# lilinitsy/skele-raytracer

Hardware: AMD Instinct MI355X
Metric: Mrays/sec + frame ms, 1920x1080 gillum=16 spheres2.scn (higher is better)
Workload: dtype f32

## Files before the change

skele_raytracer_amd/csrc/launch.h:

```cpp
#pragma once

#include <hip/hip_runtime.h>
#include <stddef.h>
#include <stdint.h>

#include "render_params.h"

enum { SKR_LEVEL0_RUN = 0, SKR_LEVEL0_BUILD, SKR_LEVEL0_REPLAY };
enum { SKR_PIX_NONE = 0, SKR_PIX_NODE, SKR_PIX_BACKGROUND, SKR_PIX_TRIANGLE };

constexpr int SKR_NODE_LEVELS_MAX = 33;
struct NodePlan {
	bool flat = false;
	int levels = 0;
	uint32_t band_nblk = 0;
	uint64_t nodes_max[SKR_NODE_LEVELS_MAX] = {};
	uint32_t cap[SKR_NODE_LEVELS_MAX] = {};
	size_t off_nodes[SKR_NODE_LEVELS_MAX] = {}, off_shade[SKR_NODE_LEVELS_MAX] = {}, off_recs[SKR_NODE_LEVELS_MAX] = {}, off_res[SKR_NODE_LEVELS_MAX] = {}, off_ixh[SKR_NODE_LEVELS_MAX] = {};
	size_t off_ctr = 0, ctr_bytes = 0, total = 0, banded = 0;
	size_t off_cls = 0, off_sums = 0;
	size_t off_girow = 0;
	int level0 = SKR_LEVEL0_RUN;
	size_t lds_leaf = 0;
	size_t lds = 0;
};

constexpr int SKR_GLEVELS_MAX = 64;
struct GPlan {
	int levels = 0;
	uint32_t band_rows = 0;
	uint64_t nodes_max[SKR_GLEVELS_MAX + 1] = {};
	uint32_t cap[SKR_GLEVELS_MAX + 1] = {};
	size_t off_nodes[SKR_GLEVELS_MAX + 1] = {}, off_recs[SKR_GLEVELS_MAX + 1] = {}, off_res[SKR_GLEVELS_MAX + 1] = {}, off_hdr[SKR_GLEVELS_MAX + 1] = {};
	size_t off_ctr = 0, ctr_bytes = 0, total = 0;
};

struct QueryTrees {
	const float4 *tree;
	const float4 *trace;
	uint32_t stride;
	int32_t nchunks;
	int32_t cones, trace_cones;
	float4 ball;
};

// ... 48 lines not shown
constexpr size_t SKR_PREFIX_LDS = ((size_t) SKR_PREFIX_WORDS * sizeof(uint32_t) + 15) & ~(size_t) 15;
static inline size_t skr_scene_kernels_lds(const RenderParams &p) { return skr_scene_lds_bytes(p) + 32 + SKR_PREFIX_LDS; }
static inline size_t skr_lights_lds_bytes(const RenderParams &p) { return ((size_t) 1 + 2 * p.n_lights) * 16; }
static inline size_t skr_lights_kernels_lds(const RenderParams &p) { return skr_lights_lds_bytes(p) + 32 + SKR_PREFIX_LDS; }

static inline uint32_t skr_tree_arity(const RenderParams &p) { return (uint32_t) (p.monte_carlo ? p.num_path_traces : 0) + (p.legacy_reflect ? 2u * (uint32_t) p.n_lights : 0u); }

struct ScratchLayout {
	size_t off = 0;
	size_t take(size_t bytes) { const size_t o = off; off += (bytes + 255) & ~(size_t) 255; return o; }
};

template <class Fits>
static uint32_t skr_largest_band(uint32_t all, Fits fits)
{
	if(fits(all)) return all;
	uint32_t lo = 1, hi = all;
	if(!fits(lo)) return 0;
	while(hi - lo > 1)
	{
		const uint32_t mid = lo + (hi - lo) / 2;
		if(fits(mid)) lo = mid;
		else hi = mid;
	}
	return lo;
}

#ifndef SKR_TRACE_BY_NODE
#define SKR_TRACE_BY_NODE 1
#endif
#ifndef SKR_TRACE_RUN
#define SKR_TRACE_RUN 2
#endif
__host__ __device__ static inline uint64_t skr_trace_header_row(uint64_t node, uint32_t j, uint32_t PP)
{
	return SKR_TRACE_BY_NODE ? (node >> 6) * PP + j : (node * PP + j) >> 6;
}
__host__ __device__ static inline uint32_t skr_trace_header_bit(uint64_t node, uint32_t j, uint32_t PP)
{
	return (uint32_t) (SKR_TRACE_BY_NODE ? node : node * PP + j) & 63u;
}
static inline uint64_t skr_trace_rows_used(uint64_t nodes, uint64_t PP) { return SKR_TRACE_BY_NODE ? (nodes + 63) / 64 * PP : (nodes * PP + 63) / 64; }
static inline uint64_t skr_trace_rows_alloc(uint64_t nodes, uint64_t PP) { return skr_trace_rows_used(nodes, PP) + 4; }
static inline uint64_t skr_trace_region_cap(uint64_t nodes, uint64_t PP) { return (skr_trace_rows_used(nodes, PP) + SKR_P1_REGIONS - 1) / SKR_P1_REGIONS * 128; }

enum SkrLeafShape { SKR_LEAF_RUNTIME = 0, SKR_LEAF_POINT1 = 1, SKR_LEAF_POINT2 = 2 };
static inline SkrLeafShape skr_leaf_shape(const RenderParams &p)
{
	if(!(p.sw.shadow_mask & SKR_SW_LEAF_SHAPE)) return SKR_LEAF_RUNTIME;
	if(p.n_tris != 0 || p.gi_index == nullptr || p.gi_wide != 0) return SKR_LEAF_RUNTIME;
	if(!p.use_shadows || p.shadow_masks == nullptr) return SKR_LEAF_RUNTIME;
	if(p.pow_steps > 7) return SKR_LEAF_RUNTIME;
	return p.n_lights == 2 ? SKR_LEAF_POINT2 : p.n_lights == 1 ? SKR_LEAF_POINT1 : SKR_LEAF_RUNTIME;
}

bool skr_plan_launch(const RenderParams &p, size_t lds_limit, LaunchPlan &lp, const GenericFeatures &f);
const char *skr_features_conflict(const GenericFeatures &f, bool legacy_reflect, bool shade_triangles, bool fog);
const char *skr_generic_variant(bool query, const GenericFeatures &f);
hipError_t skr_launch_render(const RenderParams &p, const LaunchPlan &lp, hipStream_t stream, const SkrTimingHook *hook);
hipError_t skr_launch_debug(int op, const void *d_in, void *d_out, uint32_t n, hipStream_t stream);
bool skr_nodes_plan(const RenderParams &p, size_t lds_limit, NodePlan &pl);
hipError_t skr_launch_nodes(const RenderParams &p, const NodePlan &pl, hipStream_t stream, const SkrTimingHook *hook);
hipError_t skr_nodes_level_count(const void *scratch, size_t off_ctr, int level, uint32_t *n);
bool skr_generic_plan(const RenderParams &p, GPlan &pl, bool sphere_tree = false);
hipError_t skr_launch_generic(const RenderParams &p, const GPlan &pl, hipStream_t stream, const SkrTimingHook *hook, const GenericFeatures &f, const ShadeRays *q = nullptr);
struct PrimaryKey {
// ... 65 lines not shown
```

skele_raytracer_amd/csrc/render_nodes.hip:

```cpp
#include <hip/hip_runtime.h>
#include <stdint.h>
#include <stdlib.h>
#include <string.h>

#include <vector>

#include "launch.h"
#include "wave_common.h"

namespace {

constexpr uint32_t PC_HIT0 = 1u, PC_HIT1 = 2u, PC_BLACK0 = 4u, PC_BLACK1 = 8u;
constexpr int IXH_ROWS = 3;
constexpr int NQ_CAP = 176;
constexpr int NQ_PRE = NQ_CAP - 128;
constexpr int NQ_F = 5;
constexpr int NWIN = 4;
constexpr int WIN_FLOATS = 2 * 3 * 64;
constexpr int LEAF2_WAVE_FLOATS = NQ_CAP * NQ_F + NWIN * WIN_FLOATS;

typedef const RenderParams __attribute__((address_space(4))) *LaunchArgs;
SKR_DEV const RenderParams &launch_args()
{
	LaunchArgs k = (LaunchArgs) __builtin_amdgcn_kernarg_segment_ptr();
// ... 2 lines not shown
}

SKR_DEV bool classify_child(const SceneView &sv, f3 co, f3 d, float two_a, float four_a, const BestState &s, bool &black)
{
	black = false;
	if(sv.nt > 0)
	{
		const float tmin = (s.best >= 0) ? near_root(two_a, s.b, s.D) : __builtin_inff();
		black = any_triangle_closer(sv, RayConst{co, d, two_a, four_a}, tmin);
	}
	return !black && s.best >= 0;
}

}

#ifndef SKR_TRACE_LOOP
#define SKR_TRACE_LOOP 1
#endif
#if SKR_TRACE_LOOP
#define SKR_TRACE_STRIDE gridDim.x
#else
#define SKR_TRACE_STRIDE 0x40000000u
#undef SKR_TRACE_GRID_MAX
#define SKR_TRACE_GRID_MAX 0x7fffffffu
#endif
#ifndef SKR_TRACE_WAVES
#define SKR_TRACE_WAVES 0
#endif
#if SKR_TRACE_WAVES
#define SKR_TRACE_ATTR __attribute__((amdgpu_waves_per_eu(SKR_TRACE_WAVES, SKR_TRACE_WAVES)))
#else
#define SKR_TRACE_ATTR
#endif
template <bool TRIS, bool GIM>
SKR_DEV void trace_round(const SceneView &sv, const RenderParams &p, bool valid, uint32_t node, uint32_t j, f3 co, f3 Nn, f3 nt, f3 nb, uint32_t pixel,
						 uint32_t node_id, int gi_row, uint32_t chunk, int lane, Counters &cn)
{
	const uint32_t N = (uint32_t) p.num_path_traces;
	const bool second = valid && 2u * j + 1u < N;
	bool hit0 = false, hit1 = false;
	float4 rec0 = make_float4(0, 0, 0, 0), rec1 = rec0;
	bool black0 = false, black1 = false;
	if(valid)
	{
		uint32_t rnd[4];
		philox4x32(pixel, p.aa_index, node_id, j, p.seed_lo, p.seed_hi, rnd);
		const float q1a = u31_to_unit(rnd[0]), q2a = u31_to_unit(rnd[1]), q1b = u31_to_unit(rnd[2]), q2b = u31_to_unit(rnd[3]);
		const DirPair dp = gi_direction_pair(q1a, q2a, q1b, q2b, Nn, nt, nb);
		const f3 d0 = dp.d0, d1 = dp.d1;
		cn.rays += second ? 2u : 1u;
		const RayPair rp = make_pair(d0, d1);
		BestState s0, s1;
		closest_pair<GIM>(sv, p, gi_row, co, d0, d1, second, rp, s0, s1);
		hit0 = classify_child(sv, co, d0, rp.two_a.x, rp.four_a.x, s0, black0);
		rec0 = make_float4(__uint_as_float(node), __uint_as_float((uint32_t) (s0.best & 0xffff) | ((2u * j) << 16)), q1a, q2a);
		if(second)
		{
			hit1 = classify_child(sv, co, d1, rp.two_a.y, rp.four_a.y, s1, black1);
			rec1 = make_float4(__uint_as_float(node), __uint_as_float((uint32_t) (s1.best & 0xffff) | ((2u * j + 1u) << 16)), q1b, q2b);
		}
	}
	const unsigned long long m0 = __ballot(hit0), m1 = __ballot(hit1);
	const uint32_t region = chunk & (SKR_P1_REGIONS - 1u);
	const uint32_t n0h = (uint32_t) __popcll(m0), n1h = (uint32_t) __popcll(m1);
	uint32_t base = 0;
	if(n0h + n1h != 0u)
	{
		if(lane == 0) base = atomicAdd(lc_count(p.rc_ctr, region), n0h + n1h);
		base = (uint32_t) __builtin_amdgcn_readfirstlane((int) base);
	}
	const uint32_t rec_base = region * p.rc_cap + base;
	const uint32_t rank0 = (uint32_t) lanes_below(m0), rank1 = (uint32_t) lanes_below(m1);
	if(hit0) p.rc[rec_base + rank0] = rec0;
	if(hit1) p.rc[rec_base + n0h + rank1] = rec1;
	if(TRIS)
	{
		const unsigned long long k0 = __ballot(black0), k1 = __ballot(black1);
		if(lane == 0) p.ixh[IXH_ROWS * (size_t) chunk + 2] = make_uint4((uint32_t) k0, (uint32_t) (k0 >> 32), (uint32_t) k1, (uint32_t) (k1 >> 32));
	}
	if(lane == 0)
	{
		p.ixh[IXH_ROWS * (size_t) chunk] = make_uint4(rec_base, n0h, 0u, 0u);
		p.ixh[IXH_ROWS * (size_t) chunk + 1] = make_uint4((uint32_t) m0, (uint32_t) (m0 >> 32), (uint32_t) m1, (uint32_t) (m1 >> 32));
	}
}

__host__ __device__ static inline uint32_t trace_run(uint32_t PP) { return SKR_TRACE_RUN > 0 && (uint32_t) SKR_TRACE_RUN < PP ? (uint32_t) SKR_TRACE_RUN : PP; }
__host__ __device__ static inline uint32_t trace_runs_per_block(uint32_t PP) { return (PP + trace_run(PP) - 1u) / trace_run(PP); }

#if SKR_TRACE_BY_NODE
template <bool TRIS, bool GIM>
__global__ __launch_bounds__(256) SKR_TRACE_ATTR void skr_trace_kernel(const RenderParams)
{
	extern __shared__ __align__(16) unsigned char lds_raw[];
	float4 *lds4 = reinterpret_cast<float4 *>(lds_raw);
	const RenderParams &p = launch_args();
	const uint32_t PP0 = ((uint32_t) p.num_path_traces + 1u) >> 1;
	const uint32_t items = ((*p.nd_count + 63u) >> 6) * trace_runs_per_block(PP0);
	if((uint64_t) blockIdx.x * 4u >= items) return;
	stage_scene(p, lds4, TRIS);
	const int tid = threadIdx.x, lane = tid & 63;
	const uint32_t wave = (uint32_t) uni(tid >> 6);
	Counters cn{0, 0, 0};
	for(uint32_t blk = blockIdx.x; (uint64_t) blk * 4u < items; blk += SKR_TRACE_STRIDE)
	{
		const uint32_t item = blk * 4u + wave;
		if(item >= items) break;
		uint32_t j0, j1, node;
		bool valid;
		f3 nt = mk3(0, 1, 0);
		int gi_row = -1;
		{
			const RenderParams &p = launch_args();
			const uint32_t PP = ((uint32_t) p.num_path_traces + 1u) >> 1, RPB = trace_runs_per_block(PP), RUN = trace_run(PP);
			const uint32_t B = item / RPB;
			j0 = (item - B * RPB) * RUN;
			j1 = j0 + RUN < PP ? j0 + RUN : PP;
			node = B * 64u + (uint32_t) lane;
			valid = node < *p.nd_count;
			if(valid)
			{
				const float4 *row = p.nd_src + (size_t) node * 2;
				const float4 a0 = row[0], a1 = row[1];
				const f3 co = mk3(a0.x, a0.y, a0.z), Nn = mk3(a0.w, a1.x, a1.y);
				f3 nb;
				tangent_basis(Nn, nt, nb);
				if(GIM) gi_row = p.gi_row0 ? p.gi_row0[node] : gi_origin_row(p, co);
			}
		}
		for(uint32_t j = j0; j < j1; j++)
		{
			const RenderParams &p = launch_args();
			const SceneView sv = scene_view(p, lds4, TRIS);
			f3 co = mk3(0, 0, 1), Nn = mk3(0, 0, 1);
			uint32_t pixel = 0, node_id = 0;
			if(valid)
			{
				const float4 *row = p.nd_src + (size_t) node * 2;
				const float4 a0 = row[0], a1 = row[1];
				co = mk3(a0.x, a0.y, a0.z);
				Nn = mk3(a0.w, a1.x, a1.y);
				pixel = __float_as_uint(a1.z);
				node_id = __float_as_uint(a1.w);
			}
			const f3 nb = cross3(Nn, nt);
			const uint32_t chunk = (node >> 6) * (((uint32_t) p.num_path_traces + 1u) >> 1) + j;
			trace_round<TRIS, GIM>(sv, p, valid, node, j, co, Nn, nt, nb, pixel, node_id, gi_row, (uint32_t) uni((int) chunk), lane, cn);
		}
	}
	add_counters(launch_args(), cn, (uint32_t) blockIdx.x * 4u + wave, lane);
}
#else
template <bool TRIS, bool GIM>
__global__ __launch_bounds__(256) SKR_TRACE_ATTR void skr_trace_kernel(const RenderParams)
{
	extern __shared__ __align__(16) unsigned char lds_raw[];
	float4 *lds4 = reinterpret_cast<float4 *>(lds_raw);
	const RenderParams &p = launch_args();
	const uint32_t N = (uint32_t) p.num_path_traces, PP = (N + 1u) >> 1;
	const uint64_t n_pairs = (uint64_t) *p.nd_count * PP;
	if((uint64_t) blockIdx.x * 256u >= n_pairs) return;
	stage_scene(p, lds4, TRIS);
	const int tid = threadIdx.x, lane = tid & 63;
	Counters cn{0, 0, 0};
	for(uint32_t blk = blockIdx.x; (uint64_t) blk * 256u < n_pairs; blk += SKR_TRACE_STRIDE)
	{
	const RenderParams &p = launch_args();
	const SceneView sv = scene_view(p, lds4, TRIS);
	const uint32_t chunk = blk * 4u + (uint32_t) (tid >> 6);
	const uint64_t tp = (uint64_t) chunk * 64u + (uint32_t) lane;
	const bool valid = tp < n_pairs;
	const uint32_t node = valid ? (uint32_t) (tp / PP) : 0u, j = valid ? (uint32_t) (tp - (uint64_t) node * PP) : 0u;
	f3 co = mk3(0, 0, 1), Nn = mk3(0, 0, 1), nt = mk3(0, 1, 0), nb = mk3(1, 0, 0);
	uint32_t pixel = 0, node_id = 0;
	int gi_row = -1;
	if(valid)
	{
		const float4 *row = p.nd_src + (size_t) node * 2;
		const float4 a0 = row[0], a1 = row[1];
		co = mk3(a0.x, a0.y, a0.z);
		Nn = mk3(a0.w, a1.x, a1.y);
		pixel = __float_as_uint(a1.z);
		node_id = __float_as_uint(a1.w);
		tangent_basis(Nn, nt, nb);
		if(GIM) gi_row = p.gi_row0 ? p.gi_row0[node] : gi_origin_row(p, co);
	}
	trace_round<TRIS, GIM>(sv, p, valid, node, j, co, Nn, nt, nb, pixel, node_id, gi_row, chunk, lane, cn);
	}
	add_counters(launch_args(), cn, (uint32_t) blockIdx.x * 4u + (uint32_t) (tid >> 6), lane);
}
#endif

struct Activated {
	f3 co, N, direct;
	uint32_t pixel, node_id, sph, child;
	float r1;
};

template <typename SH = RunTimeShape>
SKR_DEV Activated activate_record(const SceneView &sv, const RenderParams &p, bool act, uint32_t rec, Counters &cn)
{
	Activated a;
	a.co = a.N = mk3(0, 0, 1);
	a.direct = mk3(0, 0, 0);
	a.pixel = a.node_id = a.sph = a.child = 0;
	a.r1 = 0.0f;
	if(act)
	{
		typedef float v4f __attribute__((ext_vector_type(4)));
		const v4f n0 = __builtin_nontemporal_load(reinterpret_cast<const v4f *>(p.rc + rec));
		const uint32_t parent = __float_as_uint(n0.x), sc = __float_as_uint(n0.y);
		a.r1 = n0.z;
		a.sph = sc & 0xffffu;
		a.child = sc >> 16;
		const float4 *row = p.nd_src + (size_t) parent * 2;
		const float4 p0 = row[0], p1 = row[1];
		const f3 co0 = mk3(p0.x, p0.y, p0.z), N0 = mk3(p0.w, p1.x, p1.y);
		a.pixel = __float_as_uint(p1.z);
		const uint32_t pnode = __float_as_uint(p1.w);
		a.node_id = pnode * (uint32_t) p.num_path_traces + a.child + 1u;
		f3 nt0, nb0;
		tangent_basis(N0, nt0, nb0);
		const f3 d = gi_direction(a.r1, n0.w, N0, nt0, nb0);
		const float4 g = sv.geom[a.sph];
		const f3 ec = co0 - ld3(g);
		const float aa = dot3(d, d);
		const float b = 2 * dot3(d, ec);
		const float D = b * b - (4 * aa) * (dot3(ec, ec) - g.w);
		const float two_a = 2 * aa;
		const float t = near_root(two_a, b, D);
		const f3 P = co0 + d * t;
		a.N = normalize3(P - ld3(sv.geom[a.sph]));
		cn.hits++;
		a.direct = direct_light<false, SH>(sv, p, (int) a.sph, P, a.N, cn);
		a.co = add_scalar(P, 0.00001f);
	}
	return a;
}

#ifndef SKR_SHADE_WAVES
#define SKR_SHADE_WAVES 5
#endif
#if SKR_SHADE_WAVES
#define SKR_SHADE_ATTR __attribute__((amdgpu_waves_per_eu(SKR_SHADE_WAVES, SKR_SHADE_WAVES)))
#else
#define SKR_SHADE_ATTR
#endif
template <bool TRIS>
__global__ __launch_bounds__(256) SKR_SHADE_ATTR void skr_activate_kernel(const RenderParams p)
{
	extern __shared__ __align__(16) unsigned char lds_raw[];
	float4 *lds4 = reinterpret_cast<float4 *>(lds_raw);
	const uint32_t per_region = (p.rc_cap + 255u) / 256u;
	const uint32_t region = (uint32_t) blockIdx.x / per_region, pos0 = ((uint32_t) blockIdx.x % per_region) * 256u;
	const uint32_t cnt = *lc_count(p.rc_ctr, region);
	if(pos0 >= cnt && blockIdx.x != 0) return;
	__shared__ uint32_t s_pre[SKR_PREFIX_WORDS];
	region_prefix(p, s_pre, blockIdx.x == 0);
	if(pos0 >= cnt) return;
	const SceneView sv = stage_scene(p, lds4, TRIS);
	const uint32_t pos = pos0 + threadIdx.x;
	const bool act = pos < cnt;
	const uint32_t rec = region * p.rc_cap + pos;
	Counters cn{0, 0, 0};
	const Activated a = activate_record(sv, p, act, rec, cn);
	if(act)
	{
		const size_t n = (size_t) (s_pre[region] + pos);
		float4 *grow = p.nd_dst + n * 2, *srow = p.ns_dst + n * 2;
		grow[0] = make_float4(a.co.x, a.co.y, a.co.z, a.N.x);
		grow[1] = make_float4(a.N.y, a.N.z, __uint_as_float(a.pixel), __uint_as_float(a.node_id));
		srow[0] = make_float4(a.direct.x, a.direct.y, a.direct.z, __uint_as_float(a.sph));
		srow[1] = make_float4(a.r1, __uint_as_float(rec), __uint_as_float(a.pixel), __uint_as_float(a.node_id));
	}
	add_counters(p, cn, blockIdx.x * 4u + (threadIdx.x >> 6), threadIdx.x & 63);
}

template <bool TRIS>
__global__ __launch_bounds__(256) SKR_SHADE_ATTR void skr_shade_leaf_kernel(const RenderParams p)
{
	extern __shared__ __align__(16) unsigned char lds_raw[];
	float4 *lds4 = reinterpret_cast<float4 *>(lds_raw);
	__shared__ uint32_t prefix[SKR_PREFIX_WORDS];
	region_prefix(p, prefix, false);
	const uint32_t total = prefix[64];
	if((uint32_t) blockIdx.x * 256u >= total) return;
	const SceneView sv = stage_scene(p, lds4, TRIS);
	Counters cn{0, 0, 0};
	for(uint32_t base = (uint32_t) blockIdx.x * 256u; base < total; base += gridDim.x * 256u)
	{
		const uint32_t i = base + threadIdx.x;
		const bool act = i < total;
		uint32_t lo = 0, hi = SKR_P1_REGIONS;
		while(hi - lo > 1u)
		{
			const uint32_t mid = (lo + hi) >> 1;
			if(prefix[mid] <= (act ? i : 0u)) lo = mid;
			else hi = mid;
		}
		const uint32_t rec = lo * p.rc_cap + ((act ? i : 0u) - prefix[lo]);
		const Activated a = activate_record(sv, p, act, rec, cn);
		if(act)
		{
			const f3 tot = mk3(0, 0, 0);
			const f3 colour = (div3_const(a.direct, SKR_DIV_PI) + tot * 2.0f) * ld3(sv.kd[a.sph]);
			store3(p.res_out + (size_t) rec * 3, div3_const(colour * a.r1, SKR_DIV_PDF));
		}
	}
	add_counters(p, cn, blockIdx.x * 4u + (threadIdx.x >> 6), threadIdx.x & 63);
}

namespace {

struct Ring {
	float *base;
	int head, count;
};

SKR_DEV void ring_push(Ring &q, bool pred, f3 d, uint32_t ids, float r1)
{
	const unsigned long long m = __ballot(pred);
	if(pred)
	{
		int e = q.head + q.count + lanes_below(m);
		e -= (e >= NQ_CAP) ? NQ_CAP : 0;
		float *r = q.base + e;
		r[0 * NQ_CAP] = d.x;
		r[1 * NQ_CAP] = d.y;
		r[2 * NQ_CAP] = d.z;
		r[3 * NQ_CAP] = __uint_as_float(ids);
		r[4 * NQ_CAP] = r1;
	}
	q.count = uni(q.count + (int) __popcll(m));
}
// ... 52 lines not shown
};

}

#if defined(SKR_DIAG) && SKR_DIAG
extern "C" void skr_diag_read_nodes(unsigned long long *out, int reset)
{
	unsigned long long h[SKR_DIAG_SLOTS * 64];
	(void) hipDeviceSynchronize();
	(void) hipMemcpyFromSymbol(h, HIP_SYMBOL(skr_diag), sizeof(h));
	for(int i = 0; i < SKR_DIAG_SLOTS; i++)
	{
		out[i] = 0;
		for(int k = 0; k < 64; k++) out[i] += h[i * 64 + k];
	}
	if(reset)
	{
		memset(h, 0, sizeof(h));
		(void) hipMemcpyToSymbol(HIP_SYMBOL(skr_diag), h, sizeof(h));
	}
}
#endif
#if defined(SKR_TIMELINE) && SKR_TIMELINE
static __device__ unsigned long long skr_leaf2_times[6 * 4096];
extern "C" void skr_leaf2_times_read(unsigned long long *out)
{
	(void) hipDeviceSynchronize();
	(void) hipMemcpyFromSymbol(out, HIP_SYMBOL(skr_leaf2_times), sizeof(unsigned long long) * 6 * 4096);
}
#endif
#ifndef SKR_LEAF2_OCC
#define SKR_LEAF2_OCC 4
#endif
template <bool TRIS, bool FIRST, bool GIM, typename... SHAPE>
__global__ __launch_bounds__(256, SKR_LEAF2_OCC) void skr_leaf_kernel2(const RenderParams p)
{
	typedef typename ShapeOf<SHAPE...>::type SH;
	extern __shared__ __align__(16) unsigned char lds_raw[];
	float4 *lds4 = reinterpret_cast<float4 *>(lds_raw);
	const SceneView sv = stage_scene(p, lds4, TRIS);
	const int tid = threadIdx.x, wave = tid >> 6, lane = tid & 63;
	const uint32_t g = (uint32_t) blockIdx.x * 4u + (uint32_t) wave;
	float *wbase = reinterpret_cast<float *>(lds4 + 4 * p.n_spheres + 1 + 2 * (SH::lights > 0 ? SH::lights : p.n_lights)) + wave * LEAF2_WAVE_FLOATS;
	Ring q{wbase, 0, 0};
	float *slots = wbase + NQ_CAP * NQ_F;
	const int N = p.num_path_traces, PP = (N + 1) >> 1;
	uint32_t region = g & (SKR_P1_REGIONS - 1u);
	unsigned long long dead = 0;
	const uint32_t n_first = FIRST ? *p.nd_count : 0u;
	const uint32_t US = 64u;
	const int pl = lane, cs = 64, R = PP;
	const uint32_t units_first = (n_first + US - 1u) / US;
	Counters cn{0, 0, 0};
	STAMP_DECL;
#if defined(SKR_TIMELINE) && SKR_TIMELINE
	const unsigned long long wt_start = wall_clock64(), wc_start = __builtin_readcyclecounter();
	unsigned long long wt_first = 0, wt_last = 0;
	uint32_t wt_units = 0;
#endif
	for(;;)
	{
		uint32_t first = 0;
		int m = 0;
		bool got = false;
		for(;;)
		{
			uint32_t k = 0;
// ... 29 lines not shown
			if(live == 0ull) break;
			const unsigned long long after = region == 63u ? 0ull : (live >> (region + 1u)) << (region + 1u);
			region = (uint32_t) __builtin_ctzll(after ? after : live);
		}
		if(!got) break;
		STAMP(0);
#if defined(SKR_TIMELINE) && SKR_TIMELINE
		if(wt_units == 0) wt_first = wall_clock64();
#endif

		const bool act0 = lane < m;
		f3 co = mk3(0, 0, 1), Nn = mk3(0, 0, 1), direct1 = mk3(0, 0, 0);
		uint32_t pixel = 0, node_id = 0, out_idx = 0;
		int gi_row = -1;
		if(FIRST)
		{
			uint32_t sph0 = ~0u;
			if(act0)
			{
				const size_t nn = (size_t) (first + (uint32_t) lane);
				const float4 a0 = p.nd_src[nn * 2], a1 = p.nd_src[nn * 2 + 1], b0 = p.ns_src[nn * 2], b1 = p.ns_src[nn * 2 + 1];
				co = mk3(a0.x, a0.y, a0.z);
				Nn = mk3(a0.w, a1.x, a1.y);
				direct1 = mk3(b0.x, b0.y, b0.z);
				pixel = __float_as_uint(a1.z);
				out_idx = __float_as_uint(b1.y);
				sph0 = __float_as_uint(b0.w);
			}
			if(GIM) gi_row = gi_surface_row(p, sv, (int) sph0, co);
		}
		else
		{
			out_idx = region * p.rc_cap + first + (uint32_t) lane;
			const Activated a = activate_record<SH>(sv, p, act0, out_idx, cn);
			co = a.co;
			Nn = a.N;
			direct1 = a.direct;
			pixel = a.pixel;
			node_id = a.node_id;
			if(GIM) gi_row = gi_surface_row(p, sv, (int) a.sph, co);
		}
		const bool act = act0;
		f3 nt, nb;
		tangent_basis(Nn, nt, nb);
		STAMP(1);
		f3 acc = mk3(0, 0, 0);
		for(int jj = 0; jj < R; jj++)
		{
			const int j = jj;
			const bool second = 2 * j + 1 < N;
			float *wrow = slots + (jj & (NWIN - 1)) * WIN_FLOATS + pl;
			if(jj >= NWIN)
			{
				wave_lds_fence();
				for(int c = 0; c < 2; c++) acc = acc + mk3(wrow[(3 * c) * cs], wrow[(3 * c + 1) * cs], wrow[(3 * c + 2) * cs]);
				wave_lds_fence();
			}
			float *win = wrow;
			bool hit0 = false, hit1 = false;
			f3 d0 = mk3(0, 0, 1), d1 = mk3(0, 0, 1);
			float q1a = 0, q1b = 0;
			int s0b = 0, s1b = 0;
			if(act)
			{
				uint32_t rnd[4];
				uint32_t k0 = p.seed_lo, k1 = p.seed_hi;
				asm volatile("" : "+s"(k0), "+s"(k1));
// ... 50 lines not shown
						wave_lds_fence();
						const uint32_t head_ids = (uint32_t) uni((int) __float_as_uint(q.base[3 * NQ_CAP + q.head]));
						go = (int) (head_ids >> 23) <= jj + 1 - NWIN;
					}
				}
				if(!go) break;
				STAMP(4);
				leaf_batch<SH>(sv, p, q, slots, co, lane, q.count < 64 ? q.count : 64, cn);
				STAMP(3);
			}
			STAMP(4);
		}
		wave_lds_fence();
		for(int jr = (R > NWIN ? R - NWIN : 0); jr < R; jr++)
		{
			const float *wrow = slots + (jr & (NWIN - 1)) * WIN_FLOATS + pl;
			for(int c = 0; c < 2; c++)
				if(2 * jr + c < N) acc = acc + mk3(wrow[(3 * c) * cs], wrow[(3 * c + 1) * cs], wrow[(3 * c + 2) * cs]);
		}
		wave_lds_fence();
		if(act0)
		{
			f3 direct;
			uint32_t sph;
			float r1 = 0.0f;
			if(FIRST)
			{
				direct = direct1;
				sph = __float_as_uint(p.ns_src[(size_t) (first + (uint32_t) lane) * 2].w);
			}
			else
			{
				direct = direct1;
				const float4 r1row = p.rc[out_idx];
				r1 = r1row.z;
				sph = __float_as_uint(r1row.y) & 0xffffu;
			}
			const f3 total = acc / (float) N;
			const f3 colour = (div3_const(direct, SKR_DIV_PI) + total * 2.0f) * ld3(sv.kd[sph]);
			if(FIRST) emit_sample(p, out_idx, colour);
			else store3(p.res_out + (size_t) out_idx * 3, div3_const(colour * r1, SKR_DIV_PDF));
		}
		STAMP(5);
#if defined(SKR_TIMELINE) && SKR_TIMELINE
		wt_units++;
		wt_last = wall_clock64();
#endif
	}
#if defined(SKR_TIMELINE) && SKR_TIMELINE
	if(lane == 0 && g < 4096u)
	{
		skr_leaf2_times[6 * g] = wt_start;
		skr_leaf2_times[6 * g + 1] = wt_first;
		skr_leaf2_times[6 * g + 2] = wt_last;
		skr_leaf2_times[6 * g + 3] = wall_clock64();
		skr_leaf2_times[6 * g + 4] = wt_units;
		skr_leaf2_times[6 * g + 5] = __builtin_readcyclecounter() - wc_start;
	}
#endif
#if defined(SKR_STAMPS) && SKR_STAMPS
	if(p.counters && lane == 0)
		for(int k = 0; k < 8; k++) atomicAdd(&p.counters[4u * SKR_COUNTER_SHARDS + k], st_acc[k]);
#endif
	add_counters(p, cn, g, lane);
}

__global__ __launch_bounds__(256) void skr_finalize_kernel2(const RenderParams p)
// ... 72 lines not shown
							const float r1 = u31_to_unit(rnd[2 * c]);
							term = (code[k] & (c ? PC_BLACK1 : PC_BLACK0)) ? mk3(0, 0, 0) : div3_const(p.background * r1, SKR_DIV_PDF);
						}
						total = total + term;
					}
				}
			}
		}
	}
	const f3 direct = mk3(b0.x, b0.y, b0.z);
	const uint32_t sph = __float_as_uint(b0.w);
	total = total / (float) N;
	const f3 colour = (div3_const(direct, SKR_DIV_PI) + total * 2.0f) * ld3(p.sph_kd[sph]);
	if(p.nd_src_level0) emit_sample(p, __float_as_uint(b1.y), colour);
	else store3(p.res_out + (size_t) __float_as_uint(b1.y) * 3, div3_const(colour * b1.x, SKR_DIV_PDF));
}

#ifndef SKR_TRACE_GRID_MAX
#define SKR_TRACE_GRID_MAX 49152u
#endif
#ifndef SKR_FLAT_BELOW
#define SKR_FLAT_BELOW 1.2e7
#endif
static const uint32_t LEAF2_GRID = 256u * SKR_LEAF2_OCC;

static bool nodes_flat_wanted(const RenderParams &p)
{
	if(p.sw.flat) return p.sw.flat > 0;
	double recs = (double) p.width * p.out_rows;
	for(int k = 2; k < p.max_depth; k++) recs *= (double) p.num_path_traces;
	return recs < SKR_FLAT_BELOW;
}

static bool plan_for(const RenderParams &p, uint32_t nblk, bool flat, NodePlan &pl)
{
	const uint64_t N = (uint64_t) p.num_path_traces, PP = (N + 1) >> 1;
	pl.flat = flat;
	pl.levels = p.max_depth - 1 + (flat ? 1 : 0);
	if(pl.levels < 1 || pl.levels > SKR_NODE_LEVELS_MAX) return false;
	pl.band_nblk = nblk;
	pl.nodes_max[0] = (uint64_t) nblk * 256u;
	pl.cap[0] = 0;
	for(int L = 1; L < pl.levels; L++)
	{
		const uint64_t cap = skr_trace_region_cap(pl.nodes_max[L - 1], PP);
		if(cap * SKR_P1_REGIONS >= (1ull << 31)) return false;
		pl.cap[L] = (uint32_t) cap;
		pl.nodes_max[L] = cap * SKR_P1_REGIONS;
	}
	ScratchLayout s;
	pl.ctr_bytes = (SKR_PULL_STRIDE + LVL_CTR_WORDS * (size_t) pl.levels) * sizeof(uint32_t);
	pl.off_ctr = s.take(pl.ctr_bytes);
	for(int L = 0; L < pl.levels; L++)
	{
		const size_t n = (size_t) pl.nodes_max[L];
		if(L > 0)
		{
			pl.off_recs[L] = s.take(n * 16);
			pl.off_res[L] = s.take(n * 12 + 16);
		}
		if(L < pl.levels - 1 || pl.levels == 1)
		{
			pl.off_nodes[L] = s.take(n * 32);
			pl.off_shade[L] = s.take(n * 32);
		}
		if(L < pl.levels - 1)
		{
			pl.off_ixh[L] = s.take((size_t) skr_trace_rows_alloc(n, PP) * IXH_ROWS * 16);
		}
	}
	pl.banded = s.off - (pl.off_nodes[0]);
	pl.off_cls = s.take((size_t) nblk * 256u);
	pl.off_sums = s.take((size_t) SKR_COUNTER_SHARDS * 4 * sizeof(unsigned long long));
	pl.off_girow = s.take((size_t) nblk * 256u * sizeof(int32_t));
	pl.total = s.off;
	return true;
}

extern "C" uint32_t skr_trace_header_map(uint32_t nodes, uint32_t N, uint64_t *out, uint32_t *rows, uint32_t *bits)
{
	const uint32_t PP = (N + 1u) >> 1;
	if(out)
	{
		out[0] = skr_trace_rows_used(nodes, PP);
		out[1] = skr_trace_rows_alloc(nodes, PP);
		out[2] = skr_trace_region_cap(nodes, PP);
	}
	for(uint32_t n = 0; n < nodes && rows && bits; n++)
		for(uint32_t j = 0; j < PP; j++)
		{
			rows[(size_t) n * PP + j] = (uint32_t) skr_trace_header_row(n, j, PP);
			bits[(size_t) n * PP + j] = skr_trace_header_bit(n, j, PP);
		}
	return PP;
}

static uint64_t nodes_budget(const RenderParams &p, bool flat)
{
	return p.sw.budget_mb ? (uint64_t) p.sw.budget_mb << 20 : (flat ? 8ull : 4ull) << 30;
}

static bool plan_bands(const RenderParams &p, bool flat, NodePlan &pl)
{
	const uint32_t bx = (uint32_t) (p.width + 15) / 16, by = (p.out_rows + 15) / 16;
	const uint64_t budget = nodes_budget(p, flat);
	uint32_t nblk = skr_largest_band(bx * by, [&](uint32_t n) { return plan_for(p, n, flat, pl) && pl.banded <= budget; });
	if(nblk == 0) return false;
	if(nblk > bx) nblk = nblk / bx * bx;
	return plan_for(p, nblk, flat, pl);
}

bool skr_nodes_plan(const RenderParams &p, size_t lds_limit, NodePlan &pl)
{
	const bool forced = p.sw.pipeline == SKR_PIPE_NODES;
	if(p.sw.pipeline != SKR_PIPE_AUTO && !forced) return false;
	if(p.shade_triangles || p.legacy_reflect) return false;
	if(!(p.monte_carlo && p.n_spheres > 0 && p.n_spheres < 65536 && p.max_depth >= 2 && p.num_path_traces > 0 && p.num_path_traces <= 256)) return false;
	if(!forced && p.n_tris > 64) return false;
	pl.lds_leaf = skr_scene_lds_bytes(p) + 32 + (size_t) 4 * LEAF2_WAVE_FLOATS * sizeof(float);
	if(skr_scene_kernels_lds(p) > lds_limit) return false;
	const bool leaf_fits = pl.lds_leaf <= lds_limit;
	if(nodes_flat_wanted(p) || !leaf_fits)
	{
		const uint32_t all = (uint32_t) ((p.width + 15) / 16) * ((p.out_rows + 15) / 16);
		if(plan_bands(p, true, pl) && (p.sw.flat > 0 || !leaf_fits || pl.band_nblk >= all))
		{
			pl.lds = skr_scene_kernels_lds(p);
			return true;
		}
	}
	pl.lds = pl.lds_leaf;
	return leaf_fits && plan_bands(p, false, pl);
}

hipError_t skr_nodes_level_count(const void *scratch, size_t off_ctr, int level, uint32_t *n)
{
	const uint32_t *ctr = reinterpret_cast<const uint32_t *>(reinterpret_cast<const char *>(scratch) + off_ctr);
	if(level == 0) return hipMemcpy(n, ctr, sizeof(uint32_t), hipMemcpyDeviceToHost);
	std::vector<uint32_t> h((size_t) SKR_P1_REGIONS * SKR_PULL_STRIDE);
	const hipError_t e = hipMemcpy(h.data(), ctr + SKR_PULL_STRIDE + LVL_CTR_WORDS * (size_t) level, h.size() * sizeof(uint32_t), hipMemcpyDeviceToHost);
	if(e != hipSuccess) return e;
	uint64_t total = 0;
	for(uint32_t k = 0; k < SKR_P1_REGIONS; k++) total += h[(size_t) SKR_PULL_STRIDE * k];
	*n = (uint32_t) total;
	return hipSuccess;
}

typedef void (*LeafKernel)(const RenderParams);
template <bool FIRST>
static LeafKernel leaf_instance(const RenderParams &p)
{
	switch(skr_leaf_shape(p))
	{
	case SKR_LEAF_POINT2: return skr_leaf_kernel2<false, FIRST, true, PointLightShape<2>>;
	case SKR_LEAF_POINT1: return skr_leaf_kernel2<false, FIRST, true, PointLightShape<1>>;
	default: break;
	}
	if(p.n_tris > 0) return skr_leaf_kernel2<true, FIRST, false>;
	return p.gi_index != nullptr ? skr_leaf_kernel2<false, FIRST, true> : skr_leaf_kernel2<false, FIRST, false>;
}

template <bool FIRST>
static hipError_t launch_leaf2(const RenderParams &p, size_t lds, hipStream_t stream)
{
	const LeafKernel fn = leaf_instance<FIRST>(p);
	hipError_t e = hipFuncSetAttribute(reinterpret_cast<const void *>(fn), hipFuncAttributeMaxDynamicSharedMemorySize, (int) lds);
	if(e != hipSuccess) return e;
	hipLaunchKernelGGL(fn, dim3(LEAF2_GRID), dim3(256), lds, stream, p);
	return hipGetLastError();
}

hipError_t skr_launch_nodes(const RenderParams &p_in, const NodePlan &pl, hipStream_t stream, const SkrTimingHook *hook)
{
	RenderParams p = p_in;
	char *base = reinterpret_cast<char *>(p.node_scratch);
	uint32_t *ctr0 = reinterpret_cast<uint32_t *>(base + pl.off_ctr);
	auto lvl_ctr = [&](int L) { return ctr0 + SKR_PULL_STRIDE + LVL_CTR_WORDS * (size_t) L; };
	auto nodes = [&](int L) { return reinterpret_cast<float4 *>(base + pl.off_nodes[L]); };
	auto shade = [&](int L) { return reinterpret_cast<float4 *>(base + pl.off_shade[L]); };
	const int nsamp = p.grid_size > 0 ? p.grid_size * p.grid_size : 1;
	const size_t lds_scene = skr_scene_lds_bytes(p) + 32;
	const bool tris = p.n_tris > 0;
	const bool flat = pl.flat;
	const int D = p.max_depth, last = flat ? D - 1 : D - 2;
	const uint32_t blocks_x = (uint32_t) (p.width + 15) / 16, blocks = blocks_x * ((p.out_rows + 15) / 16);
	p.blocks_x = blocks_x;
	p.qctr = ctr0;
	hipError_t e = hipSuccess;
	for(int s = 0; s < nsamp; s++)
	{
		p.aa_index = (uint32_t) s;
		for(uint32_t blk0 = 0; blk0 < blocks; blk0 += pl.band_nblk)
		{
			const bool timed = hook && s == nsamp - 1 && blk0 == 0;
			p.band_blk0 = blk0;
			p.band_nblk = blocks - blk0 < pl.band_nblk ? blocks - blk0 : pl.band_nblk;
			p.nd_dst = nodes(0);
			p.ns_dst = shade(0);
			uint8_t *cls = reinterpret_cast<uint8_t *>(base + pl.off_cls);
			unsigned long long *sums = reinterpret_cast<unsigned long long *>(base + pl.off_sums);
			int32_t *const gi_row0 = pl.level0 != SKR_LEVEL0_RUN ? reinterpret_cast<int32_t *>(base + pl.off_girow) : nullptr;
			p.gi_row0 = gi_row0;
			if(pl.level0 == SKR_LEVEL0_REPLAY)
			{
				e = hipMemsetAsync(ctr0 + SKR_PULL_STRIDE, 0, pl.ctr_bytes - SKR_PULL_STRIDE * sizeof(uint32_t), stream);
				if(e == hipSuccess) e = skr_launch_primary_replay(p, cls, sums, stream);
			}
			else
			{
				e = hipMemsetAsync(ctr0, 0, pl.ctr_bytes, stream);
				if(e == hipSuccess)
					e = pl.level0 == SKR_LEVEL0_BUILD ? skr_launch_primary_build(p, dim3(p.band_nblk), lds_scene, cls, sums, stream)
													  : skr_launch_primary(p, dim3(p.band_nblk), lds_scene, stream);
			}
			if(e != hipSuccess) return e;
			if(D == 2 && !flat)
			{
				p.nd_src = nodes(0);
				p.ns_src = shade(0);
				p.nd_src_level0 = 1;
				p.nd_count = ctr0;
				p.rc_ctr = lvl_ctr(0);
				if(timed) skr_hook_start(hook, stream);
				e = launch_leaf2<true>(p, pl.lds_leaf, stream);
				if(timed) skr_hook_stop(hook, stream);
				if(e != hipSuccess) return e;
				continue;
			}
			for(int L = 1; L <= last; L++)
			{
				p.nd_src = nodes(L - 1);
				p.ns_src = shade(L - 1);
				p.nd_src_level0 = L == 1;
				p.gi_row0 = L == 1 ? gi_row0 : nullptr;
				p.nd_count = L == 1 ? ctr0 : lc_prefix_host(lvl_ctr(L - 1));
				p.rc = reinterpret_cast<float4 *>(base + pl.off_recs[L]);
				p.rc_cap = pl.cap[L];
				p.rc_ctr = lvl_ctr(L);
				p.ixh = reinterpret_cast<uint4 *>(base + pl.off_ixh[L - 1]);
#if SKR_TRACE_BY_NODE
				const uint64_t wg_t = ((pl.nodes_max[L - 1] + 63) / 64 * trace_runs_per_block(((uint32_t) p.num_path_traces + 1u) >> 1) + 3) / 4;
#else
				const uint64_t wg_t = (pl.nodes_max[L - 1] * (uint64_t) ((p.num_path_traces + 1) >> 1) + 255) / 256;
#endif
				const unsigned grid_t = (unsigned) (wg_t < SKR_TRACE_GRID_MAX ? wg_t : SKR_TRACE_GRID_MAX);
				if(flat && L == last && timed) skr_hook_start(hook, stream);
				if(tris) hipLaunchKernelGGL((skr_trace_kernel<true, false>), dim3(grid_t), dim3(256), lds_scene, stream, p);
				else if(p.gi_index) hipLaunchKernelGGL((skr_trace_kernel<false, true>), dim3(grid_t), dim3(256), lds_scene, stream, p);
				else hipLaunchKernelGGL((skr_trace_kernel<false, false>), dim3(grid_t), dim3(256), lds_scene, stream, p);
				if(L < last)
				{
					p.nd_dst = nodes(L);
					p.ns_dst = shade(L);
					const unsigned grid_a = SKR_P1_REGIONS * ((pl.cap[L] + 255u) / 256u);
					if(tris) hipLaunchKernelGGL(skr_activate_kernel<true>, dim3(grid_a), dim3(256), lds_scene, stream, p);
					else hipLaunchKernelGGL(skr_activate_kernel<false>, dim3(grid_a), dim3(256), lds_scene, stream, p);
				}
			}
			p.res_out = reinterpret_cast<float *>(base + pl.off_res[last]);
			if(flat)
			{
				const uint64_t wg = (pl.nodes_max[last] + 255) / 256;
				const unsigned grid_s = (unsigned) (wg < 16384 ? wg : 16384);
				if(tris) hipLaunchKernelGGL(skr_shade_leaf_kernel<true>, dim3(grid_s), dim3(256), lds_scene, stream, p);
				else hipLaunchKernelGGL(skr_shade_leaf_kernel<false>, dim3(grid_s), dim3(256), lds_scene, stream, p);
				if(timed) skr_hook_stop(hook, stream);
			}
			else
			{
				if(timed) skr_hook_start(hook, stream);
				e = launch_leaf2<false>(p, pl.lds_leaf, stream);
				if(timed) skr_hook_stop(hook, stream);
				if(e != hipSuccess) return e;
			}
			for(int L = last - 1; L >= 0; L--)
			{
				p.nd_src = nodes(L);
				p.ns_src = shade(L);
				p.nd_src_level0 = L == 0;
				p.nd_count = L == 0 ? ctr0 : lc_prefix_host(lvl_ctr(L));
				p.ixh = reinterpret_cast<uint4 *>(base + pl.off_ixh[L]);
				p.res_in = reinterpret_cast<const float *>(base + pl.off_res[L + 1]);
				p.res_out = L == 0 ? nullptr : reinterpret_cast<float *>(base + pl.off_res[L]);
				hipLaunchKernelGGL(skr_finalize_kernel2, dim3((unsigned) ((pl.nodes_max[L] + 255) / 256)), dim3(256), 0, stream, p);
			}
			e = hipGetLastError();
			if(e != hipSuccess) return e;
		}
	}
	if(p.grid_size > 0) return skr_launch_resolve(p, stream);
	return hipSuccess;
}
```

Before: 70890.

## Store ray direction and quadratic terms in wide hit records to skip recomputation

Hit records written by the trace kernel grow from one float4 to two. They now also hold the ray direction, the quadratic b term and the discriminant. The activation path reads these back instead of rebuilding the tangent basis, regenerating the GI direction and recomputing the sphere intersection terms. In exchange, record memory and write/read traffic double, and because the planner tries wide layout first and falls back to narrow only if the budget fails, wide records can shrink the band size. A plan-map export function is also added.

```diff
diff --git a/skele_raytracer_amd/csrc/launch.h b/skele_raytracer_amd/csrc/launch.h
--- a/skele_raytracer_amd/csrc/launch.h
+++ b/skele_raytracer_amd/csrc/launch.h
@@ -11,6 +11,7 @@
 
 constexpr int SKR_NODE_LEVELS_MAX = 33;
 struct NodePlan {
+	bool wide = false;
 	bool flat = false;
 	int levels = 0;
 	uint32_t band_nblk = 0;
@@ -125,6 +126,11 @@
 #ifndef SKR_TRACE_RUN
 #define SKR_TRACE_RUN 2
 #endif
+#ifndef SKR_WIDE_RECORDS
+#define SKR_WIDE_RECORDS 1
+#endif
+__host__ __device__ constexpr int skr_rec_rows(bool wide) { return wide ? 2 : 1; }
+static inline size_t skr_records_bytes(uint64_t records, bool wide) { return (size_t) records * (size_t) skr_rec_rows(wide) * 16; }
 __host__ __device__ static inline uint64_t skr_trace_header_row(uint64_t node, uint32_t j, uint32_t PP)
 {
 	return SKR_TRACE_BY_NODE ? (node >> 6) * PP + j : (node * PP + j) >> 6;
diff --git a/skele_raytracer_amd/csrc/render_nodes.hip b/skele_raytracer_amd/csrc/render_nodes.hip
--- a/skele_raytracer_amd/csrc/render_nodes.hip
+++ b/skele_raytracer_amd/csrc/render_nodes.hip
@@ -58,7 +58,7 @@
 #else
 #define SKR_TRACE_ATTR
 #endif
-template <bool TRIS, bool GIM>
+template <bool TRIS, bool GIM, bool WIDE>
 SKR_DEV void trace_round(const SceneView &sv, const RenderParams &p, bool valid, uint32_t node, uint32_t j, f3 co, f3 Nn, f3 nt, f3 nb, uint32_t pixel,
 						 uint32_t node_id, int gi_row, uint32_t chunk, int lane, Counters &cn)
 {
@@ -66,6 +66,8 @@
 	const bool second = valid && 2u * j + 1u < N;
 	bool hit0 = false, hit1 = false;
 	float4 rec0 = make_float4(0, 0, 0, 0), rec1 = rec0;
+	float4 ray0 = rec0, ray1 = rec0;
+	constexpr int ROWS = skr_rec_rows(WIDE);
 	bool black0 = false, black1 = false;
 	if(valid)
 	{
@@ -79,11 +81,13 @@
 		BestState s0, s1;
 		closest_pair<GIM>(sv, p, gi_row, co, d0, d1, second, rp, s0, s1);
 		hit0 = classify_child(sv, co, d0, rp.two_a.x, rp.four_a.x, s0, black0);
-		rec0 = make_float4(__uint_as_float(node), __uint_as_float((uint32_t) (s0.best & 0xffff) | ((2u * j) << 16)), q1a, q2a);
+		rec0 = make_float4(__uint_as_float(node), __uint_as_float((uint32_t) (s0.best & 0xffff) | ((2u * j) << 16)), q1a, WIDE ? s0.D : q2a);
+		if(WIDE) ray0 = make_float4(d0.x, d0.y, d0.z, s0.b);
 		if(second)
 		{
 			hit1 = classify_child(sv, co, d1, rp.two_a.y, rp.four_a.y, s1, black1);
-			rec1 = make_float4(__uint_as_float(node), __uint_as_float((uint32_t) (s1.best & 0xffff) | ((2u * j + 1u) << 16)), q1b, q2b);
+			rec1 = make_float4(__uint_as_float(node), __uint_as_float((uint32_t) (s1.best & 0xffff) | ((2u * j + 1u) << 16)), q1b, WIDE ? s1.D : q2b);
+			if(WIDE) ray1 = make_float4(d1.x, d1.y, d1.z, s1.b);
 		}
 	}
 	const unsigned long long m0 = __ballot(hit0), m1 = __ballot(hit1);
@@ -97,8 +101,16 @@
 	}
 	const uint32_t rec_base = region * p.rc_cap + base;
 	const uint32_t rank0 = (uint32_t) lanes_below(m0), rank1 = (uint32_t) lanes_below(m1);
-	if(hit0) p.rc[rec_base + rank0] = rec0;
-	if(hit1) p.rc[rec_base + n0h + rank1] = rec1;
+	if(hit0)
+	{
+		p.rc[(size_t) (rec_base + rank0) * ROWS] = rec0;
+		if(WIDE) p.rc[(size_t) (rec_base + rank0) * ROWS + 1] = ray0;
+	}
+	if(hit1)
+	{
+		p.rc[(size_t) (rec_base + n0h + rank1) * ROWS] = rec1;
+		if(WIDE) p.rc[(size_t) (rec_base + n0h + rank1) * ROWS + 1] = ray1;
+	}
 	if(TRIS)
 	{
 		const unsigned long long k0 = __ballot(black0), k1 = __ballot(black1);
@@ -115,7 +127,7 @@
 __host__ __device__ static inline uint32_t trace_runs_per_block(uint32_t PP) { return (PP + trace_run(PP) - 1u) / trace_run(PP); }
 
 #if SKR_TRACE_BY_NODE
-template <bool TRIS, bool GIM>
+template <bool TRIS, bool GIM, bool WIDE>
 __global__ __launch_bounds__(256) SKR_TRACE_ATTR void skr_trace_kernel(const RenderParams)
 {
 	extern __shared__ __align__(16) unsigned char lds_raw[];
@@ -171,13 +183,13 @@
 			}
 			const f3 nb = cross3(Nn, nt);
 			const uint32_t chunk = (node >> 6) * (((uint32_t) p.num_path_traces + 1u) >> 1) + j;
-			trace_round<TRIS, GIM>(sv, p, valid, node, j, co, Nn, nt, nb, pixel, node_id, gi_row, (uint32_t) uni((int) chunk), lane, cn);
+			trace_round<TRIS, GIM, WIDE>(sv, p, valid, node, j, co, Nn, nt, nb, pixel, node_id, gi_row, (uint32_t) uni((int) chunk), lane, cn);
 		}
 	}
 	add_counters(launch_args(), cn, (uint32_t) blockIdx.x * 4u + wave, lane);
 }
 #else
-template <bool TRIS, bool GIM>
+template <bool TRIS, bool GIM, bool WIDE>
 __global__ __launch_bounds__(256) SKR_TRACE_ATTR void skr_trace_kernel(const RenderParams)
 {
 	extern __shared__ __align__(16) unsigned char lds_raw[];
@@ -211,7 +223,7 @@
 		tangent_basis(Nn, nt, nb);
 		if(GIM) gi_row = p.gi_row0 ? p.gi_row0[node] : gi_origin_row(p, co);
 	}
-	trace_round<TRIS, GIM>(sv, p, valid, node, j, co, Nn, nt, nb, pixel, node_id, gi_row, chunk, lane, cn);
+	trace_round<TRIS, GIM, WIDE>(sv, p, valid, node, j, co, Nn, nt, nb, pixel, node_id, gi_row, chunk, lane, cn);
 	}
 	add_counters(launch_args(), cn, (uint32_t) blockIdx.x * 4u + (uint32_t) (tid >> 6), lane);
 }
@@ -223,7 +235,7 @@
 	float r1;
 };
 
-template <typename SH = RunTimeShape>
+template <bool WIDE, typename SH = RunTimeShape>
 SKR_DEV Activated activate_record(const SceneView &sv, const RenderParams &p, bool act, uint32_t rec, Counters &cn)
 {
 	Activated a;
@@ -234,25 +246,39 @@
 	if(act)
 	{
 		typedef float v4f __attribute__((ext_vector_type(4)));
-		const v4f n0 = __builtin_nontemporal_load(reinterpret_cast<const v4f *>(p.rc + rec));
+		const v4f n0 = __builtin_nontemporal_load(reinterpret_cast<const v4f *>(p.rc + (size_t) rec * skr_rec_rows(WIDE)));
 		const uint32_t parent = __float_as_uint(n0.x), sc = __float_as_uint(n0.y);
 		a.r1 = n0.z;
 		a.sph = sc & 0xffffu;
 		a.child = sc >> 16;
 		const float4 *row = p.nd_src + (size_t) parent * 2;
 		const float4 p0 = row[0], p1 = row[1];
-		const f3 co0 = mk3(p0.x, p0.y, p0.z), N0 = mk3(p0.w, p1.x, p1.y);
+		const f3 co0 = mk3(p0.x, p0.y, p0.z);
 		a.pixel = __float_as_uint(p1.z);
 		const uint32_t pnode = __float_as_uint(p1.w);
 		a.node_id = pnode * (uint32_t) p.num_path_traces + a.child + 1u;
+		f3 d;
+		float b, D, aa;
+		if(WIDE)
+		{
+		const v4f n1 = __builtin_nontemporal_load(reinterpret_cast<const v4f *>(p.rc + (size_t) rec * skr_rec_rows(WIDE) + 1));
+		d = mk3(n1.x, n1.y, n1.z);
+		b = n1.w;
+		D = n0.w;
+		aa = dot3(d, d);
+		}
+		else
+		{
+		const f3 N0 = mk3(p0.w, p1.x, p1.y);
 		f3 nt0, nb0;
 		tangent_basis(N0, nt0, nb0);
-		const f3 d = gi_direction(a.r1, n0.w, N0, nt0, nb0);
+		d = gi_direction(a.r1, n0.w, N0, nt0, nb0);
 		const float4 g = sv.geom[a.sph];
 		const f3 ec = co0 - ld3(g);
-		const float aa = dot3(d, d);
-		const float b = 2 * dot3(d, ec);
-		const float D = b * b - (4 * aa) * (dot3(ec, ec) - g.w);
+		aa = dot3(d, d);
+		b = 2 * dot3(d, ec);
+		D = b * b - (4 * aa) * (dot3(ec, ec) - g.w);
+		}
 		const float two_a = 2 * aa;
 		const float t = near_root(two_a, b, D);
 		const f3 P = co0 + d * t;
@@ -272,7 +298,7 @@
 #else
 #define SKR_SHADE_ATTR
 #endif
-template <bool TRIS>
+template <bool TRIS, bool WIDE>
 __global__ __launch_bounds__(256) SKR_SHADE_ATTR void skr_activate_kernel(const RenderParams p)
 {
 	extern __shared__ __align__(16) unsigned char lds_raw[];
@@ -289,7 +315,7 @@
 	const bool act = pos < cnt;
 	const uint32_t rec = region * p.rc_cap + pos;
 	Counters cn{0, 0, 0};
-	const Activated a = activate_record(sv, p, act, rec, cn);
+	const Activated a = activate_record<WIDE>(sv, p, act, rec, cn);
 	if(act)
 	{
 		const size_t n = (size_t) (s_pre[region] + pos);
@@ -302,7 +328,7 @@
 	add_counters(p, cn, blockIdx.x * 4u + (threadIdx.x >> 6), threadIdx.x & 63);
 }
 
-template <bool TRIS>
+template <bool TRIS, bool WIDE>
 __global__ __launch_bounds__(256) SKR_SHADE_ATTR void skr_shade_leaf_kernel(const RenderParams p)
 {
 	extern __shared__ __align__(16) unsigned char lds_raw[];
@@ -325,7 +351,7 @@
 			else hi = mid;
 		}
 		const uint32_t rec = lo * p.rc_cap + ((act ? i : 0u) - prefix[lo]);
-		const Activated a = activate_record(sv, p, act, rec, cn);
+		const Activated a = activate_record<WIDE>(sv, p, act, rec, cn);
 		if(act)
 		{
 			const f3 tot = mk3(0, 0, 0);
@@ -444,7 +470,7 @@
 #ifndef SKR_LEAF2_OCC
 #define SKR_LEAF2_OCC 4
 #endif
-template <bool TRIS, bool FIRST, bool GIM, typename... SHAPE>
+template <bool TRIS, bool FIRST, bool GIM, bool WIDE, typename... SHAPE>
 __global__ __launch_bounds__(256, SKR_LEAF2_OCC) void skr_leaf_kernel2(const RenderParams p)
 {
 	typedef typename ShapeOf<SHAPE...>::type SH;
@@ -540,7 +566,7 @@
 		else
 		{
 			out_idx = region * p.rc_cap + first + (uint32_t) lane;
-			const Activated a = activate_record<SH>(sv, p, act0, out_idx, cn);
+			const Activated a = activate_record<WIDE, SH>(sv, p, act0, out_idx, cn);
 			co = a.co;
 			Nn = a.N;
 			direct1 = a.direct;
@@ -657,7 +683,7 @@
 			else
 			{
 				direct = direct1;
-				const float4 r1row = p.rc[out_idx];
+				const float4 r1row = p.rc[(size_t) out_idx * skr_rec_rows(WIDE)];
 				r1 = r1row.z;
 				sph = __float_as_uint(r1row.y) & 0xffffu;
 			}
@@ -796,8 +822,9 @@
 	return recs < SKR_FLAT_BELOW;
 }
 
-static bool plan_for(const RenderParams &p, uint32_t nblk, bool flat, NodePlan &pl)
-{
+static bool plan_for(const RenderParams &p, uint32_t nblk, bool flat, bool wide, NodePlan &pl)
+{
+	pl.wide = wide;
 	const uint64_t N = (uint64_t) p.num_path_traces, PP = (N + 1) >> 1;
 	pl.flat = flat;
 	pl.levels = p.max_depth - 1 + (flat ? 1 : 0);
@@ -820,7 +847,7 @@
 		const size_t n = (size_t) pl.nodes_max[L];
 		if(L > 0)
 		{
-			pl.off_recs[L] = s.take(n * 16);
+			pl.off_recs[L] = s.take(skr_records_bytes(n, wide));
 			pl.off_res[L] = s.take(n * 12 + 16);
 		}
 		if(L < pl.levels - 1 || pl.levels == 1)
@@ -864,14 +891,41 @@
 	return p.sw.budget_mb ? (uint64_t) p.sw.budget_mb << 20 : (flat ? 8ull : 4ull) << 30;
 }
 
+static bool plan_bands(const RenderParams &p, bool flat, NodePlan &pl);
+extern "C" int skr_nodes_plan_map(int32_t width, uint32_t rows, int32_t N, int32_t depth, int32_t flat, int32_t budget_mb, uint32_t nblk, uint64_t *out)
+{
+	RenderParams p{};
+	p.width = width;
+	p.out_rows = rows;
+	p.num_path_traces = N;
+	p.max_depth = depth;
+	p.sw.budget_mb = budget_mb;
+	NodePlan pl;
+	if(!(nblk ? plan_for(p, nblk, flat != 0, true, pl) : plan_bands(p, flat != 0, pl))) return 0;
+	const uint64_t head[16] = {(uint64_t) pl.levels, pl.band_nblk, pl.total, pl.banded, pl.off_ctr, pl.ctr_bytes, pl.off_cls, pl.off_sums,
+							   pl.off_girow, skr_records_bytes(1, pl.wide), 0, 0, 0, 0, 0, 0};
+	memcpy(out, head, sizeof head);
+	for(int L = 0; L < SKR_NODE_LEVELS_MAX; L++)
+	{
+		const uint64_t row[8] = {pl.nodes_max[L], pl.cap[L], pl.off_nodes[L], pl.off_shade[L], pl.off_recs[L], pl.off_res[L], pl.off_ixh[L],
+								 L < pl.levels ? skr_records_bytes(pl.nodes_max[L], pl.wide) : 0};
+		memcpy(out + 16 + 8 * L, row, sizeof row);
+	}
+	return 1;
+}
+
 static bool plan_bands(const RenderParams &p, bool flat, NodePlan &pl)
 {
 	const uint32_t bx = (uint32_t) (p.width + 15) / 16, by = (p.out_rows + 15) / 16;
 	const uint64_t budget = nodes_budget(p, flat);
-	uint32_t nblk = skr_largest_band(bx * by, [&](uint32_t n) { return plan_for(p, n, flat, pl) && pl.banded <= budget; });
-	if(nblk == 0) return false;
-	if(nblk > bx) nblk = nblk / bx * bx;
-	return plan_for(p, nblk, flat, pl);
+	for(int wide = SKR_WIDE_RECORDS ? 1 : 0; wide >= 0; wide--)
+	{
+		uint32_t nblk = skr_largest_band(bx * by, [&](uint32_t n) { return plan_for(p, n, flat, wide != 0, pl) && pl.banded <= budget; });
+		if(nblk == 0) continue;
+		if(nblk > bx) nblk = nblk / bx * bx;
+		return plan_for(p, nblk, flat, wide != 0, pl);
+	}
+	return false;
 }
 
 bool skr_nodes_plan(const RenderParams &p, size_t lds_limit, NodePlan &pl)
@@ -911,23 +965,25 @@
 }
 
 typedef void (*LeafKernel)(const RenderParams);
+template <bool FIRST, bool WIDE>
+static LeafKernel leaf_instance(const RenderParams &p)
+{
+	switch(skr_leaf_shape(p))
+	{
+	case SKR_LEAF_POINT2: return skr_leaf_kernel2<false, FIRST, true, WIDE, PointLightShape<2>>;
+	case SKR_LEAF_POINT1: return skr_leaf_kernel2<false, FIRST, true, WIDE, PointLightShape<1>>;
+	default: break;
+	}
+	if(p.n_tris > 0) return skr_leaf_kernel2<true, FIRST, false, WIDE>;
+	return p.gi_index != nullptr ? skr_leaf_kernel2<false, FIRST, true, WIDE> : skr_leaf_kernel2<false, FIRST, false, WIDE>;
+}
+
 template <bool FIRST>
-static LeafKernel leaf_instance(const RenderParams &p)
-{
-	switch(skr_leaf_shape(p))
-	{
-	case SKR_LEAF_POINT2: return skr_leaf_kernel2<false, FIRST, true, PointLightShape<2>>;
-	case SKR_LEAF_POINT1: return skr_leaf_kernel2<false, FIRST, true, PointLightShape<1>>;
-	default: break;
-	}
-	if(p.n_tris > 0) return skr_leaf_kernel2<true, FIRST, false>;
-	return p.gi_index != nullptr ? skr_leaf_kernel2<false, FIRST, true> : skr_leaf_kernel2<false, FIRST, false>;
-}
-
-template <bool FIRST>
-static hipError_t launch_leaf2(const RenderParams &p, size_t lds, hipStream_t stream)
-{
-	const LeafKernel fn = leaf_instance<FIRST>(p);
+static hipError_t launch_leaf2(const RenderParams &p, bool wide, size_t lds, hipStream_t stream)
+{
+	LeafKernel fn;
+	if constexpr(FIRST) fn = leaf_instance<true, false>(p);
+	else fn = wide ? leaf_instance<false, true>(p) : leaf_instance<false, false>(p);
 	hipError_t e = hipFuncSetAttribute(reinterpret_cast<const void *>(fn), hipFuncAttributeMaxDynamicSharedMemorySize, (int) lds);
 	if(e != hipSuccess) return e;
 	hipLaunchKernelGGL(fn, dim3(LEAF2_GRID), dim3(256), lds, stream, p);
@@ -986,7 +1042,7 @@
 				p.nd_count = ctr0;
 				p.rc_ctr = lvl_ctr(0);
 				if(timed) skr_hook_start(hook, stream);
-				e = launch_leaf2<true>(p, pl.lds_leaf, stream);
+				e = launch_leaf2<true>(p, pl.wide, pl.lds_leaf, stream);
 				if(timed) skr_hook_stop(hook, stream);
 				if(e != hipSuccess) return e;
 				continue;
@@ -1009,16 +1065,18 @@
 #endif
 				const unsigned grid_t = (unsigned) (wg_t < SKR_TRACE_GRID_MAX ? wg_t : SKR_TRACE_GRID_MAX);
 				if(flat && L == last && timed) skr_hook_start(hook, stream);
-				if(tris) hipLaunchKernelGGL((skr_trace_kernel<true, false>), dim3(grid_t), dim3(256), lds_scene, stream, p);
-				else if(p.gi_index) hipLaunchKernelGGL((skr_trace_kernel<false, true>), dim3(grid_t), dim3(256), lds_scene, stream, p);
-				else hipLaunchKernelGGL((skr_trace_kernel<false, false>), dim3(grid_t), dim3(256), lds_scene, stream, p);
+				const LeafKernel trace = tris       ? (pl.wide ? skr_trace_kernel<true, false, true> : skr_trace_kernel<true, false, false>)
+										 : p.gi_index ? (pl.wide ? skr_trace_kernel<false, true, true> : skr_trace_kernel<false, true, false>)
+													  : (pl.wide ? skr_trace_kernel<false, false, true> : skr_trace_kernel<false, false, false>);
+				hipLaunchKernelGGL(trace, dim3(grid_t), dim3(256), lds_scene, stream, p);
 				if(L < last)
 				{
 					p.nd_dst = nodes(L);
 					p.ns_dst = shade(L);
 					const unsigned grid_a = SKR_P1_REGIONS * ((pl.cap[L] + 255u) / 256u);
-					if(tris) hipLaunchKernelGGL(skr_activate_kernel<true>, dim3(grid_a), dim3(256), lds_scene, stream, p);
-					else hipLaunchKernelGGL(skr_activate_kernel<false>, dim3(grid_a), dim3(256), lds_scene, stream, p);
+					const LeafKernel activate = tris ? (pl.wide ? skr_activate_kernel<true, true> : skr_activate_kernel<true, false>)
+													 : (pl.wide ? skr_activate_kernel<false, true> : skr_activate_kernel<false, false>);
+					hipLaunchKernelGGL(activate, dim3(grid_a), dim3(256), lds_scene, stream, p);
 				}
 			}
 			p.res_out = reinterpret_cast<float *>(base + pl.off_res[last]);
@@ -1026,14 +1084,15 @@
 			{
 				const uint64_t wg = (pl.nodes_max[last] + 255) / 256;
 				const unsigned grid_s = (unsigned) (wg < 16384 ? wg : 16384);
-				if(tris) hipLaunchKernelGGL(skr_shade_leaf_kernel<true>, dim3(grid_s), dim3(256), lds_scene, stream, p);
-				else hipLaunchKernelGGL(skr_shade_leaf_kernel<false>, dim3(grid_s), dim3(256), lds_scene, stream, p);
+				const LeafKernel shade_leaf = tris ? (pl.wide ? skr_shade_leaf_kernel<true, true> : skr_shade_leaf_kernel<true, false>)
+												   : (pl.wide ? skr_shade_leaf_kernel<false, true> : skr_shade_leaf_kernel<false, false>);
+				hipLaunchKernelGGL(shade_leaf, dim3(grid_s), dim3(256), lds_scene, stream, p);
 				if(timed) skr_hook_stop(hook, stream);
 			}
 			else
 			{
 				if(timed) skr_hook_start(hook, stream);
-				e = launch_leaf2<false>(p, pl.lds_leaf, stream);
+				e = launch_leaf2<false>(p, pl.wide, pl.lds_leaf, stream);
 				if(timed) skr_hook_stop(hook, stream);
 				if(e != hipSuccess) return e;
 			}
```

After: 71710, median of 6. 1.2% higher.
